# surftemp/cae_tools

Hardware: AMD Instinct MI355X
Metric: train images/sec (16x16->256x256, batch 64) (higher is better)
Workload: dtype f32

## Files before the change

cae_tools_amd/_lib.py:

```python
import ctypes as C
import os

_HERE = os.path.dirname(os.path.abspath(__file__))
LIB_PATH = os.path.join(_HERE, "csrc", "libcae_hip.so")


class CaeError(RuntimeError):
    pass


class LayerSpecC(C.Structure):
    _fields_ = [(n, C.c_int32) for n in ("in_c", "in_h", "in_w", "out_c", "out_h", "out_w", "k_h", "k_w",
                                          "stride", "output_padding")]


class TensorInfoC(C.Structure):
    _fields_ = [("name", C.c_char * 96), ("arena", C.c_int32), ("ndim", C.c_int32), ("shape", C.c_int64 * 4),
                ("offset", C.c_int64), ("numel", C.c_int64)]


class ProfileRecC(C.Structure):
    _fields_ = [("name", C.c_char * 48), ("layer", C.c_int32), ("reserved", C.c_int32), ("micros", C.c_double),
                ("bytes", C.c_double)]

# ... 35 lines not shown
    "cae_adam_step": (C.c_int, [_P]),
    "cae_forward_backward_sync": (C.c_int, [_P, C.c_int, _P, C.c_int, C.c_int, C.c_int, ALLREDUCE_FN, _P]),
    "cae_dp_unique_id": (C.c_int, [_P]),
    "cae_dp_init": (C.c_int, [_P, C.c_int, C.c_int, _P]),
    "cae_dp_shutdown": (C.c_int, [_P]),
    "cae_dp_info": (C.c_int, [_P, C.POINTER(C.c_int), C.POINTER(C.c_int), C.POINTER(C.c_int)]),
    "cae_dp_set_overlap": (C.c_int, [_P, C.c_int]),
    "cae_dp_broadcast_state": (C.c_int, [_P, C.c_int, C.c_int]),
    "cae_dp_train_step": (C.c_int, [_P, C.c_int, _P, C.c_int, C.c_int, C.c_int]),
    "cae_dp_train_steps": (C.c_int, [_P, C.c_int, _P, C.c_int, C.c_int, C.c_int, C.c_int]),
    "cae_dp_eval_steps": (C.c_int, [_P, C.c_int, _P, C.c_int, C.c_int, C.c_int]),
    "cae_dp_read_losses": (C.c_int, [_P, C.c_int, C.c_int, C.POINTER(C.c_double)]),
    "cae_eval_step": (C.c_int, [_P, C.c_int, _P, C.c_int]),
    "cae_score": (C.c_int, [_P, _P, C.c_int, _P]),
    "cae_encode": (C.c_int, [_P, _P, C.c_int, _P]),
    "cae_decode": (C.c_int, [_P, _P, C.c_int, _P]),
    "cae_read_losses": (C.c_int, [_P, C.c_int, C.c_int, C.POINTER(C.c_double)]),
    "cae_loss_slots": (C.c_int, [_P]),
    "cae_sync": (C.c_int, [_P]),
    "cae_graph_count": (C.c_int, [_P]),
    "cae_graph_captures": (C.c_int64, [_P]),
    "cae_debug_read": (C.c_int64, [_P, C.c_char_p, C.c_int, _P, C.c_int64]),
    "cae_debug_plan": (C.c_int, [_P, C.c_int, C.c_int, C.c_char_p, C.c_int64]),
    "cae_profile_begin": (C.c_int, [_P]),
    "cae_debug_launch_floor": (C.c_int, [_P, C.c_int, C.POINTER(C.c_double)]),
    "cae_profile_end": (C.c_int, [_P, C.POINTER(ProfileRecC), C.c_int]),
    "cae_trace_range_push": (C.c_int, [C.c_char_p]),
    "cae_trace_range_pop": (C.c_int, []),
    "cae_scan_f32": (C.c_int, [_P, C.c_int64, _P, C.POINTER(C.c_double)]),
    "cae_normalise_pack": (C.c_int, [_P, C.c_int64, C.c_int, C.c_int64, _P, C.c_int, C.c_int, C.c_float,
                                     C.c_float, C.c_int, _P]),
    "cae_normalise_pack_rows": (C.c_int, [_P, C.c_int64, C.c_int, C.c_int64, _P, C.c_int, C.c_int, C.c_float,
                                          C.c_float, C.c_int, _P, _P]),
    "cae_invert_permutation": (C.c_int, [_P, C.c_int64, _P, _P]),
    "cae_denormalise_f64": (C.c_int, [_P, C.c_int64, C.c_double, C.c_double, _P, _P]),
    "cae_bswap32": (C.c_int, [_P, C.c_int64, _P]),
    "cae_metric_sums": (C.c_int, [_P, _P, _P, C.c_int64, C.c_int64, C.c_double, C.c_double, _P, _P]),
    "cae_case_measures_workspace_bytes": (C.c_int64, [C.c_int64, C.c_int64]),
    "cae_case_measures": (C.c_int, [_P, C.c_int, C.c_int64, _P, C.c_int, C.c_int64, C.c_int64, C.c_int64, _P, _P,
                                    C.c_int64, _P]),
    "cae_case_range_workspace_bytes": (C.c_int64, [C.c_int64, C.c_int64]),
    "cae_case_range": (C.c_int, [_P, C.c_int, C.c_int64, _P, C.c_int, C.c_int64, C.c_int64, C.c_int64, _P, _P, C.c_int64,
                                 _P]),
    "cae_render_cases": (C.c_int, [_P, C.c_int, C.c_int64, _P, C.c_int, C.c_int64, _P, C.c_int64, C.c_int64, C.c_int64,
                                   C.c_int64, C.c_double, C.c_double, C.c_int, _P, _P]),
    "cae_pixel_sums_workspace_bytes": (C.c_int64, [C.c_int64, C.c_int64, C.c_int64]),
# ... 142 lines not shown
```

cae_tools_amd/csrc/engine.hip:

```cpp
#include <hip/hip_runtime.h>

#include <dlfcn.h>

#include <algorithm>
#include <cmath>
#include <cstdio>
#include <cstdlib>
#include <cstring>
#include <map>
#include <string>
#include <tuple>
#include <vector>

#include "cae_hip.h"
#include "kernels_generic.h"
#include "kernels_stateless.h"
#include "kernels_spectra.h"
#include "kernels_ssim.h"
#include "kernels_baseline.h"
#include "kernels_hist.h"
#include "kernels_strata.h"
#include "kernels_fss.h"
#include "kernels_s2.h"
#include "kernels_last.h"
// ... 209 lines not shown
    for (auto& L : e->dec)
        if (L.has_bn) e->bn_saved_off[L.bn_index] = carve((int64_t)L.cout * 2 * sizeof(float));
    const int64_t mb = max_batch;
    for (auto& L : e->enc) {
        L.act_off = carve(mb * L.out_elems() * 4);
        L.grad_off = carve(mb * L.out_elems() * 4);
    }
    for (int i = 0; i < 4; i++) {
        e->fc[i].act_off = carve(mb * e->fc[i].nout * 4);
        e->fc[i].grad_off = carve(mb * e->fc[i].nout * 4);
    }
    for (auto& L : e->dec) {
        if (!L.has_bn) continue;
        L.act_off = carve(mb * L.out_elems() * 4);
        L.grad_off = carve(mb * L.out_elems() * 4);
    }
    e->off_glast = carve(mb * e->dec.back().out_elems() * 4);
    e->off_xbatch = carve((mb * e->enc[0].in_elems() + e->enc[0].cout) * 4);
    if (variational) {
        e->off_vz = carve(mb * latent_size * 4);
        e->off_vgz = carve(mb * latent_size * 4);
        e->off_zlast = carve(mb * e->dec.back().out_elems() * 4);
    }
    e->ws_need = carve.top;
    for (auto& L : e->enc)
        if (L.cin > e->max_channels) e->max_channels = L.cin;
    for (auto& L : e->dec)
        if (L.cin > e->max_channels) e->max_channels = L.cin;
    if (lds_bytes(e->max_channels, e->max_channels) > 60 * 1024) {
        delete e;
        return fail(CAE_ERR_ARG, "channel count %d exceeds the LDS constant table", e->max_channels);
    }
    *out = e;
    return CAE_OK;
}

void cae_engine_destroy(cae_engine* e) {
    if (!e) return;
    e->drop_graphs();
    (void)cae_dp_shutdown(e);
    delete e;
}

int64_t cae_param_count(const cae_engine* e) { return e ? e->tab.n_param : 0; }
int64_t cae_buffer_count(const cae_engine* e) { return e ? e->tab.n_buf : 0; }
int cae_tensor_count(const cae_engine* e) { return e ? e->tab.count() : 0; }
// ... 28 lines not shown
        e->lr_stale = true;
    }
    e->stream = (hipStream_t)hip_stream;
    return CAE_OK;
}

int cae_set_graph_mode(cae_engine* e, int enabled) {
    if (!e) return fail(CAE_ERR_ARG, "null engine");
    e->graph_mode = enabled != 0;
    if (!e->graph_mode) e->drop_graphs();
    return CAE_OK;
}

int cae_set_capture_only(cae_engine* e, int enabled) {
    if (!e) return fail(CAE_ERR_ARG, "null engine");
    e->capture_only = enabled != 0;
    return CAE_OK;
}

int cae_set_kernel_mode(cae_engine* e, int specialised) {
    if (!e) return fail(CAE_ERR_ARG, "null engine");
    const int ctb = (specialised & 2) ? 0x7fffffff : e->ctbwd_auto;
    const bool gather = (specialised & 4) != 0;
    if (e->use_s2 != ((specialised & 1) != 0) || ctb != e->ctbwd_mask || gather != e->gather_fwd) e->drop_graphs();
    e->use_s2 = (specialised & 1) != 0;
    e->ctbwd_mask = ctb;
    e->gather_fwd = gather;
    return CAE_OK;
}

int cae_set_hyper(cae_engine* e, double lr, double beta1, double beta2, double eps, double weight_decay) {
    if (!e) return fail(CAE_ERR_ARG, "null engine");
    Hyper h{lr, beta1, beta2, eps, weight_decay};
    if (h.beta1 != e->hp.beta1 || h.beta2 != e->hp.beta2 || h.eps != e->hp.eps || h.wd != e->hp.wd) e->drop_graphs();
    e->hp = h;
    e->lr_stale = true;
    return push_lr(e);
}

int cae_set_lr(cae_engine* e, double lr) {
    if (!e) return fail(CAE_ERR_ARG, "null engine");
    e->hp.lr = lr;
    e->lr_stale = true;
    return push_lr(e);
}

int cae_set_dataset(cae_engine* e, int which, const float* x, const float* t, int64_t n) {
    if (!e || which < 0 || which > 1 || !x || n < 1) return fail(CAE_ERR_ARG, "cae_set_dataset: bad argument");
    if (e->ds_x[which] != x || e->ds_t[which] != t) e->drop_graphs();
    e->ds_x[which] = x;
// ... 619 lines not shown
```

cae_tools_amd/csrc/engine_choose.h:

```cpp
#pragma once

namespace {


#define S2_SHAPES(X) X(2, 1) X(4, 2) X(8, 4) X(6, 3)
#define S2_KERNELS(X, CI, CO) X(CI, CO, 3, 3) X(CI, CO, 4, 4) X(CI, CO, 3, 4) X(CI, CO, 4, 3)

template <int CI, int CO, int KH, int KW>
struct S2Shape { static constexpr int cin = CI, cout = CO, kh = KH, kw = KW; };

template <class F>
auto s2_for_shape(const ConvLayer& L, F fn) {
#define ONE(CI, CO, KH_, KW_) \
    if (L.cin == CI && L.cout == CO && L.kh == KH_ && L.kw == KW_) return fn(S2Shape<CI, CO, KH_, KW_>{});
#define PAIR(CI, CO) S2_KERNELS(ONE, CI, CO)
    S2_SHAPES(PAIR)
#undef PAIR
#undef ONE
    return false;
}

bool s2_shape_ok(const ConvLayer& L) { return L.transposed && L.stride == 2 && s2_for_shape(L, [](auto) { return true; }); }

bool s2_eligible(const cae_engine* e, const ConvLayer& L) { return e->use_s2 && L.sh_w >= 0 && s2_shape_ok(L); }
// ... 413 lines not shown
    if (rows_ok(e, L, l)) return DF_ROWS;
    if (s2_eligible(e, L)) return DF_S2;
    if (e->use_s2 && !last && L.stride == 2 && L.kh <= 4 && L.kw <= 4) {
        CtFwd c;
        int waves = 0;
        size_t lds = 0;
        return ct_fwd_plan(e, B, L, l, c, waves, lds) ? DF_CT_LDS : DF_IG;
    }
    return DF_UP;
}

DecBwdK choose_dec_bwd(const cae_engine* e, const ConvLayer& L, int l, int B, bool external_loss) {
    const bool last = l + 1 == (int)e->dec.size();
    if (last && !external_loss && last_fused_ok(e, L)) return DB_FUSED_LAST;
    if (rows_ok(e, L, l)) return DB_ROWS;
    if (s2_eligible(e, L)) return DB_S2;
    if (e->use_s2) {
        CtBwdPlan p;
        return ct_bwd_plan(e, B, L, l, p) ? DB_CT_LDS : DB_IG;
    }
    return DB_GENERIC;
}

bool enc_conv0_fits_adam(const cae_engine* e, const StepArgs& a, const ConvLayer& L) {
    return e->use_s2 && !a.syncing() && a.world == 1 && L.cout <= 64 &&
           (int64_t)L.cin * L.cout * L.kh * L.kw <= 4096 && (int64_t)a.batch * L.hout * L.wout < kDivSmallMaxN &&
           L.hout * L.wout < kDivSmallMaxD && L.in_elems() < (1 << 24) && L.out_elems() < (1 << 24) &&
           (int64_t)a.batch * L.in_elems() < (1 << 30) && (int64_t)a.batch * L.out_elems() < (1 << 30) &&
           e->bn_stat_off[L.bn_index] == e->off_zero_begin;
}

bool enc_conv0_in_adam_ok(const cae_engine* e, const StepArgs& a, const ConvLayer& L) {
    return a.adam_follows && e->x_published && enc_conv0_fits_adam(e, a, L);
}

bool linear_bwd_burst(const cae_engine* e, int i) {
    const int K = e->fc[i].nout;
    return i > 0 && K % 4 == 0 && K >= 128 && (K / 4 + 3) / 4 <= kBurstSteps;
}

const char* head_staging(const HeadArgs& h) {
    const int per = h.enc[0].cin * h.enc[0].hin * h.enc[0].win;
    if (per & 3) return "scalar";
    return h.B * (per >> 2) <= 4 * kHeadThreads ? "direct" : "gather4";
}

// ... 105 lines not shown
                     t.sp_d[2].per, t.sp_w[0].lg, t.sp_w[0].per, t.sp_w[1].lg, t.sp_w[1].per, t.sp_w[2].lg, t.sp_w[2].per, lds);
        } else {
            snprintf(line, sizeof line, "tail bwd=layers why=%s\n", why);
        }
        s += line;
        for (int i = 3; tr && !tail_fused && i >= 0; i--) {
            if (e->use_s2) snprintf(line, sizeof line, "fc%d bwd=pair burst=%d\n", i, (int)linear_bwd_burst(e, i));
            else snprintf(line, sizeof line, "fc%d bwd=generic\n", i);
            s += line;
        }
    }
    if (tr) {
        const bool in_adam = head_fused && enc_conv0_fits_adam(e, a, e->enc[0]);
        snprintf(line, sizeof line, "enc conv0=%s inner=%s\n", in_adam ? "adam" : "own",
                 e->enc.size() < 2 ? "-" : (e->use_s2 && !a.syncing() ? "pair" : "layers"));
        s += line;
    }
    if ((int64_t)s.size() + 1 > out_bytes)
        return fail(CAE_ERR_ARG, "cae_debug_plan: the report needs %zu bytes, got %lld", s.size() + 1, (long long)out_bytes);
    memcpy(out, s.c_str(), s.size() + 1);
    return CAE_OK;
}

}
```

cae_tools_amd/csrc/engine_launch.h:

```cpp
#pragma once

namespace {


template <class K, class A>
void s2_go(K kernel, A a, int ex, int ey, int tw, int th, int cap, hipStream_t s) {
    a.tiles_x = (ex + tw - 1) / tw;
    a.tiles_y = (ey + th - 1) / th;
    a.total_tiles = a.B * a.tiles_x * a.tiles_y;
    hipLaunchKernelGGL(kernel, dim3(a.total_tiles < cap ? a.total_tiles : cap), dim3(256), 0, s, a);
}

template <int CIN, int COUT, int KH, int KW>
bool s2_fwd_launch(const S2Fwd& a, S2FwdPick p, hipStream_t s) {
    const int px = ((a.OW + 1) / 2 + 1) / 2, py = ((a.OH + 1) / 2 + 1) / 2;
    const int qx = (a.OW + 1) / 2, qy = (a.OH + 1) / 2;
    switch (p.k) {
        case S2F_CS:
            if constexpr (CIN * COUT * KH * KW > 80 && (256 / COUT) % 64 == 0) {
                constexpr int PIX = 256 / COUT;
                if (p.tw == 64) s2_go(k_s2_fwd_cs<CIN, COUT, KH, KW, 64>, a, qx, qy, 64, PIX / 64, kS2FwdCap, s);
                else s2_go(k_s2_fwd_cs<CIN, COUT, KH, KW, 32>, a, qx, qy, 32, PIX / 32, kS2FwdCap, s);
                return true;
            }
// ... 287 lines not shown
    const ConvLayer& L = c.L;
    S2Last f = zeroed<S2Last>();
    f.B = a.batch; f.H = L.hin; f.W = L.win; f.OH = L.hout; f.OW = L.wout;
    f.in = c.ain.p; f.w = e->params + L.w_off; f.bias = e->params + L.b_off;
    f.target = e->ds_t[a.which]; f.perm = a.perm; f.use_cursor = a.use_cursor ? 1 : 0;
    f.st = e->state(); f.losses = e->losses();
    f.inv_count = (float)(1.0 / ((double)a.global_batch * L.cout * L.hout * L.wout));
    f.bias_acc = e->sgacc() + L.sh_b; f.wacc = e->sgacc() + L.sh_w; f.acc_stride = e->segs.n;
    f.bn_in = c.prod.P ? bn_of(e, *c.prod.P, BN_BATCH, (double)a.bn_batch * c.prod.P->hout * c.prod.P->wout, 1) : bn_none();
    f.gin = c.prod.gin; f.stats_in = c.prod.stats_in;
    ProfScope _p(e, "s2_convt_last_fused", c.l, bytes_bwd(a.batch, L, true, false));
    return last_fused_dispatch(L, f, e->stream) ? CAE_OK : fail(CAE_ERR_STATE, "decoder layer %d: no k_s2_last_fused kernel for the chosen variant", c.l);
}

void bwd_rows(cae_engine* e, const StepArgs& a, const ConvBwd& c) {
    const ConvLayer& L = c.L;
    S2Rows f = zeroed<S2Rows>();
    f.B = a.batch; f.H = L.hin; f.W = L.win; f.OH = L.hout; f.OW = L.wout;
    f.g = c.gy.p; f.yout = c.gy.q; f.bn_out = c.bng;
    f.ain = c.ain.p; f.bn_in = c.prod.bn_prev;
    f.w = e->params + L.w_off; f.wacc = e->sgacc() + L.sh_w; f.wacc_stride = e->segs.n;
    f.gin = c.prod.gin; f.stats_in = c.prod.stats_in;
    f.bg = bn_grad_out(e, L, a);
    ProfScope _p(e, "s2_convt_bwd", c.l, bytes_bwd(a.batch, L, false, false));
    rows_bwd_launch(L, f, e->stream);
}

int bwd_s2(cae_engine* e, const StepArgs& a, const ConvBwd& c) {
    const ConvLayer& L = c.L;
    S2Bwd f = zeroed<S2Bwd>();
    f.B = a.batch; f.H = L.hin; f.W = L.win; f.OH = L.hout; f.OW = L.wout;
    f.g = c.gy.p; f.yout = c.gy.q; f.bn_out = c.bng;
    f.ain = c.ain.p; f.bn_in = c.prod.bn_prev;
    f.w = e->params + L.w_off; f.wacc = e->sgacc() + L.sh_w; f.wacc_stride = e->segs.n;
    f.gin = c.prod.gin; f.stats_in = c.prod.stats_in;
    f.bg = bn_grad_out(e, L, a);
    ProfScope _p(e, "s2_convt_bwd", c.l, bytes_bwd(a.batch, L, c.last, false));
    return s2_bwd_dispatch(L, f, e->stream) ? CAE_OK : fail(CAE_ERR_STATE, "decoder layer %d: no k_s2_bwd kernel for the chosen variant", c.l);
}

int bwd_ct_lds(cae_engine* e, const StepArgs& a, const ConvBwd& c) {
    const ConvLayer& L = c.L;
    CtBwdPlan cp;
    (void)ct_bwd_plan(e, a.batch, L, c.l, cp);
    CtBwd f = zeroed<CtBwd>();
    f.B = a.batch; f.Cin = L.cin; f.H = L.hin; f.W = L.win; f.Cout = L.cout; f.OH = L.hout; f.OW = L.wout;
    f.imgs = cp.imgs; f.wstr = cp.wstr; f.bands = cp.bands; f.hb = cp.hb;
    f.g = c.gy.p; f.yout = c.gy.q; f.bn_out = c.bng;
    f.ain = c.ain.p; f.bn_in = c.prod.bn_prev;
    f.w = e->params + L.w_off;
    f.wacc = L.sh_w >= 0 ? e->sgacc() + L.sh_w : e->gradacc() + L.w_off;
    f.wacc_stride = L.sh_w >= 0 ? e->segs.n : 0;
    f.gin = c.prod.gin; f.stats_prev = c.prod.stats_in;
    f.bg = bn_grad_out(e, L, a);
    ProfScope _p(e, "ct_convt_bwd", c.l, bytes_bwd(a.batch, L, c.last, c.l == 0));
    if (cae_internal::ctbwd_launch(&f, sizeof f, (unsigned)cp.groups, (unsigned)(L.cin / 16), (unsigned)cp.parts, cp.lds_launch, e->stream))
        return fail(CAE_ERR_ARG, "k_ct_bwd_lds: argument layout mismatch");
    return CAE_OK;
}

void bwd_ig(cae_engine* e, const StepArgs& a, const ConvBwd& c) {
    const ConvLayer& L = c.L;
    const int B = a.batch;
    const IgBwdPlan p = ig_bwd_plan(L, B);
    IgWgrad fw = zeroed<IgWgrad>();
    fw.B = B; fw.Cin = L.cin; fw.H = L.hin; fw.W = L.win; fw.Cout = L.cout; fw.OH = L.hout; fw.OW = L.wout;
    fw.KH = L.kh; fw.KW = L.kw; fw.S = L.stride;
    fw.ain = c.ain.p; fw.bn_in = c.prod.bn_prev; fw.g = c.gy.p; fw.yout = c.gy.q; fw.bn_out = c.bng;
    fw.wacc = e->gradacc() + L.w_off;
    fw.bg = bn_grad_out(e, L, a);
    fw.ksteps_per_block = p.per;
    IgDgrad fd = zeroed<IgDgrad>();
    fd.B = B; fd.Cin = L.cin; fd.H = L.hin; fd.W = L.win; fd.Cout = L.cout; fd.OH = L.hout; fd.OW = L.wout;
    fd.KH = L.kh; fd.KW = L.kw; fd.S = L.stride;
    fd.g = c.gy.p; fd.yout = c.gy.q; fd.bn_out = c.bng; fd.w = e->params + L.w_off;
    fd.gin = c.prod.gin; fd.yprev = c.prod.yprev; fd.bn_prev = c.prod.bn_prev; fd.stats_prev = c.prod.stats_in;
    fd.ksplit = p.ksplit; fd.tiles_per_wave = p.tiles_per_wave;
// ... 59 lines not shown
        gd.epi = GE_STORE;
    } else if (i > 0) {
        const FcLayer& G = e->fc[i - 1];
        gd.C = e->fptr(G.grad_off); gd.H = e->fptr(G.act_off);
        gd.epi = G.relu ? GE_RELU_MASK : GE_STORE;
    } else {
        gd.C = e->fptr(P.grad_off); gd.H = e->fptr(P.act_off);
        gd.epi = GE_BN_MASK; gd.bn_c = bni; gd.hw_c = hw; gd.stats_c = e->bn_stats(P.bn_index);
        lds = gemm_lds(P.cout);
    }
    const int tiles_d = ((gd.M + 15) / 16) * ((gd.N + 15) / 16);
    if (i == 0) {
        gw.M = F.nin + 1; gw.N = F.nout; gw.K = B;
        gw.A = in; gw.sa_m = 1; gw.sa_k = F.nin;
        gw.B = gout; gw.sb_k = F.nout; gw.sb_n = 1;
        gw.epi = GE_ACC64_T; gw.ones_col = 0; gw.ones_row = 1;
        gw.bn_a = bni; gw.hw_a = hw; gw.bn_a_by_row = 1;
    }
    {
        const int tiles_w = ((gw.M + 15) / 16) * ((gw.N + 15) / 16);
        ProfScope _p(e, "linear_bwd_pair_mfma", i, bytes_lin_bwd_pair(B, F));
        const bool burst = linear_bwd_burst(e, i);
        if (burst && gemm16_burst_lds(gd.K) > lds) lds = gemm16_burst_lds(gd.K);
        hipLaunchKernelGGL(k_gemm16_pair, dim3(tiles_w + tiles_d), dim3(256), lds, e->stream, gw, gd, tiles_w, burst ? 1 : 0);
    }
    if (i == 2 && e->variational) {
        if (!e->hooks.reparam_bwd) return fail(CAE_ERR_STATE, "trunk engine without a reparameterisation hook");
        e->hooks.reparam_bwd(e->hooks.user, e->stream, e->fptr(e->off_vgz), e->fptr(e->fc[1].act_off), B, e->latent,
                             e->fptr(e->fc[1].grad_off));
    }
    return CAE_OK;
}

void linear_bwd_generic(cae_engine* e, const StepArgs& a, int i, const ConvLayer& P) {
    const FcLayer& F = e->fc[i];
    const int B = a.batch, hw = P.hout * P.wout;
    hipStream_t s = e->stream;
    const float* gout = e->fptr(F.grad_off);
    const float* in = linear_in(e, i, P);
    BnDesc bni = i == 0 ? bn_of(e, P, BN_SAVED, 0, 0) : bn_none();
    {
        ProfScope _p(e, "linear_wgrad", i, f4((double)B * (F.nin + F.nout)) + 8.0 * F.nin * F.nout);
        hipLaunchKernelGGL(k_lin_wgrad, dim3(grid1((int64_t)F.nin * F.nout)), dim3(256),
                           lds_bytes(i == 0 ? P.cout : 0, 0), s, B, F.nin, F.nout, gout, in, bni, hw,
                           e->gradacc() + F.w_off, e->gradacc() + F.b_off);
    }
    ProfScope _p(e, "linear_dgrad", i, f4((double)B * (2.0 * F.nin + F.nout) + (double)F.nin * F.nout));
// ... 66 lines not shown
```

cae_tools_amd/csrc/engine_state.h:

```cpp
#pragma once

namespace {

constexpr float kBnEps = 1e-5f;
constexpr float kBnMomentum = 0.1f;
constexpr int kLossSlots = 1 << 16;

int64_t align_up(int64_t v, int64_t a) { return (v + a - 1) / a * a; }

template <class T>
T zeroed() {
    T t;
    memset(&t, 0, sizeof t);
    return t;
}

struct ConvLayer {
    bool transposed;
    int cin, hin, win, cout, hout, wout, kh, kw, stride, opad;
    bool has_bn;
    int bn_index;
    int64_t w_off, b_off, gamma_off, beta_off;
    int64_t rm_off, rv_off;
    int64_t act_off, grad_off;
// ... 29 lines not shown
    int64_t ws_need = 0;

    float *params = nullptr, *grads = nullptr, *m = nullptr, *v = nullptr, *bufs = nullptr;
    char* ws = nullptr;
    hipStream_t stream = nullptr;
    Hyper hp{1e-3, 0.9, 0.999, 1e-8, 1e-5};
    const float* ds_x[2] = {nullptr, nullptr};
    const float* ds_t[2] = {nullptr, nullptr};
    int64_t ds_n[2] = {0, 0};
    bool graph_mode = true;
    bool lr_stale = true;
    long long captures = 0;
    bool capture_only = false;
    bool use_s2 = true;
    bool variational = false;
    int64_t off_vz = 0, off_vgz = 0, off_zlast = 0;
    cae_internal::TrunkHooks hooks{nullptr, nullptr, nullptr};
    bool gather_fwd = false;
    int ctbwd_mask = 0;
    int ctbwd_auto = 0;
    int64_t off_xbatch = 0;
    bool x_published = false;
    AdamConv0 c0_pending{};
    bool profiling = false;
    struct ProfRec { const char* name; int layer; double bytes; hipEvent_t e0, e1; };
    std::vector<ProfRec> prof;
    std::map<std::tuple<int, int, int, int, const void*, int, int, int, int, int>, hipGraphExec_t> graphs;

    int dp_world = 0, dp_rank = 0;
    RcclApi::comm_t dp_comm = nullptr;
    hipStream_t comm_stream = nullptr;
    hipEvent_t ev_fork = nullptr, ev_join = nullptr;
    bool dp_graph_ok = true;
    bool dp_overlap = true;
    std::vector<int> sync_order;
    size_t sync_pos = 0;
    int64_t bucket_split = 0;

    StepState* state() const { return reinterpret_cast<StepState*>(ws + off_state); }
    double* losses() const { return reinterpret_cast<double*>(ws + off_losses); }
    double* gradacc() const { return reinterpret_cast<double*>(ws + off_gradacc); }
    double* sgacc() const { return reinterpret_cast<double*>(ws + off_sgacc); }
    ShardSegs shard_segs() const {
        ShardSegs r = segs;
        r.base = sgacc();
        return r;
// ... 221 lines not shown
```

cae_tools_amd/csrc/kernels_ctbwd.h:

```cpp
#pragma once
#include <type_traits>

#include "device_common.h"

namespace cae {

struct CtBwd {
    int B, Cin, H, W, Cout, OH, OW;
    int imgs;
    int bands, hb;
    int wstr;
    const float* g;
    const float* yout;
    BnDesc bn_out;
    const float* ain;
    BnDesc bn_in;
    const float* w;
    float* gin;
    double* stats_prev;
    double* wacc;
    long long wacc_stride;
    BnGradOut bg;
};

constexpr int kCtbThreads = 512;
constexpr int kCtbWaves = kCtbThreads / 64;
constexpr int kCtbG4 = 7;
constexpr int kCtbA4 = 2;
constexpr int kCtbW4 = 3;
constexpr int kCtbKChunk = 64;

inline size_t ct_bwd_lds_bytes(int Cin, int Cout, int imgs, int HW, int OHW, int wstr) {
    size_t floats = 32 * (size_t)kCtbWaves;
    floats += 4 * (size_t)(Cin + Cout);
    floats += (size_t)imgs * Cout * OHW;
    floats += (size_t)imgs * 16 * HW;
    floats += 16 * (size_t)wstr;
    floats += 3 * (size_t)imgs * HW;
    floats += (size_t)kCtbWaves * 16 * 17;
    return (floats + 8) * sizeof(float);
}

#ifdef CAE_CTBWD_KERNEL
template <bool BAND>
__device__ __forceinline__ void ct_bwd_body(const CtBwd& a) {
// ... 240 lines not shown
                    ok[u] = p < pend;
                    const int pc = ok[u] ? p : pbeg;
                    ia[u] = pos_a[pc];
                    ig[u] = pos_g[pc];
                }
                float va[8], vb[8];
#pragma unroll
                for (int u = 0; u < 8; u++) {
                    va[u] = ar[ia[u]];
                    vb[u] = gb[ig[u]];
                }
#pragma unroll
                for (int u = 0; u < 8; u++) {
                    float x = va[u];
                    if (act) x = fmaxf(0.f, fmaf(x - kin.x, kin.y, kin.z));
                    va[u] = ok[u] ? x : 0.f;
                }
#pragma unroll
                for (int u = 0; u < 8; u += 2) {
                    acc = __builtin_amdgcn_mfma_f32_16x16x4f32(va[u], vb[u], acc, 0, 0, 0);
                    acc1 = __builtin_amdgcn_mfma_f32_16x16x4f32(va[u + 1], vb[u + 1], acc1, 0, 0, 0);
                }
            }
            if (n_ok) {
#pragma unroll
                for (int j = 0; j < 4; j++) acc_add<ACC_GRAD>(&wacc_sh[(size_t)(cb * 16 + 4 * q + j) * N + n], (double)(acc[j] + acc1[j]));
            }
        }
    }
    if (a.stats_prev) {
#pragma unroll
        for (int cc = 0; cc < 4; cc++) {
            float t1 = s1[cc], t2 = s2[cc];
            t1 += dpp_f<0xB1>(t1);  t2 += dpp_f<0xB1>(t2);
            t1 += dpp_f<0x4E>(t1);  t2 += dpp_f<0x4E>(t2);
            t1 += dpp_f<0x141>(t1); t2 += dpp_f<0x141>(t2);
            t1 += dpp_f<0x140>(t1); t2 += dpp_f<0x140>(t2);
            if (pl == 0) {
                lstat[wv * 32 + 2 * (4 * cg + cc)] = t1;
                lstat[wv * 32 + 2 * (4 * cg + cc) + 1] = t2;
            }
        }
        __syncthreads();
        if (tid < 32) {
            const int c = cb * 16 + (tid >> 1);
            const int shard = (blockIdx.x + blockIdx.y + blockIdx.z) & (kStatShards - 1);
            double t = 0.0;
// ... 19 lines not shown
```

cae_tools_amd/csrc/kernels_gemm.h:

```cpp
#pragma once
#include "device_common.h"

namespace cae {

enum GemmEpi : int {
    GE_STORE = 0,
    GE_RELU_MASK = 1,
    GE_BN_MASK = 2,
    GE_ACC64 = 3,
    GE_ACC64_T = 4
};

struct GemmArgs {
    int M, N, K;
    const float* A; long long sa_m, sa_k;
    const float* B; long long sb_k, sb_n;
    float* C; long long sc_m, sc_n;
    int epi;
    const float* bias;
    int relu;
    const float* H;
    BnDesc bn_a;
    int hw_a;
    int bn_a_by_row;
// ... 174 lines not shown
    __syncthreads();
    if (wv != 0 || cn >= g.N) return;
#pragma unroll
    for (int j = 0; j < 4; j++) {
        const int cm = tm * 16 + q * 4 + j;
        if (cm >= g.M) continue;
        float v = part[j * 64 + lane] + part[256 + j * 64 + lane] + part[512 + j * 64 + lane] + part[768 + j * 64 + lane];
        const long long off = (long long)cm * g.sc_m + (long long)cn * g.sc_n;
        if (g.epi == GE_STORE) {
            v += bias;
            if (g.relu) v = fmaxf(v, 0.f);
        } else {
            v = hmask[j] > 0.f ? v : 0.f;
        }
        g.C[off] = v;
    }
}

__global__ void __launch_bounds__(256) k_gemm16(GemmArgs g) {
    extern __shared__ double lds_d[];
    gemm16_body(g, blockIdx.x, lds_d);
}

__global__ void __launch_bounds__(256) k_gemm16_pair(GemmArgs a, GemmArgs b, int na, int b_burst) {
    kernarg_warm<2 * sizeof(GemmArgs) + 8>();
    extern __shared__ double lds_d[];
    if ((int)blockIdx.x < na) gemm16_body(a, blockIdx.x, lds_d);
    else if (b_burst) gemm16_burst_body(b, blockIdx.x - na, lds_d);
    else gemm16_body(b, blockIdx.x - na, lds_d);
}

}
```

cae_tools_amd/csrc/kernels_rows.h:

```cpp
#pragma once
#include "kernels_last.h"

namespace cae {

struct S2Rows {
    int B, H, W, OH, OW;
    int QH;
    int bands;
    int groups;
    const float* g;
    const float* yout;
    BnDesc bn_out;
    const float* ain;
    BnDesc bn_in;
    const float* w;
    float* gin;
    double* stats_in;
    double* wacc;
    int wacc_stride;
    BnGradOut bg;
};

template <int CIN, int CT, int COUT, int KH, int KW, int HB, int IMGS, int D>
__global__ void __launch_bounds__(256) __attribute__((amdgpu_waves_per_eu(1, 2))) k_s2_bwd_rows(S2Rows a) {
    kernarg_warm<sizeof(S2Rows)>();
    constexpr int CS = CIN / CT;
    constexpr int NB = 4 / CS;
    constexpr int LW = 64 / IMGS;
    constexpr int NACC = CT * COUT * KH * KW;
    constexpr int NRED = NACC + 2 * CT;
    constexpr int NR = HB + 1;
    static_assert(CS * NB == 4 && CS * CT == CIN, "four waves");
    static_assert(KH == 3 && KW == 3, "3x3 stride-2 kernels");
    static_assert(CIN <= 8 && COUT <= 8, "one lane per (channel, shard) in the BatchNorm prologue");
    __shared__ float redf[4 * NRED];
    __shared__ __attribute__((aligned(16))) float wscr[4 * kWsumScratch];
    __shared__ float xch[NB > 1 ? 4 * CT * 64 : 1];
    __shared__ __attribute__((aligned(16))) float wl[CIN * COUT * 12];

    const int tid = threadIdx.x, lane = tid & 63;
    const int wv = __builtin_amdgcn_readfirstlane(tid >> 6);
    const int cgrp = wv % CS, bsel = wv / CS;
    const int c0 = cgrp * CT;
// ... 240 lines not shown
            }
        }
    }

    {
        float red[NRED];
#pragma unroll
        for (int i = 0; i < NACC; i++) red[i] = dw[i];
#pragma unroll
        for (int c = 0; c < CT; c++) {
            red[NACC + 2 * c] = d1[c];
            red[NACC + 2 * c + 1] = d2[c];
        }
        wave_sums_lds<NRED>(red, wscr + wv * kWsumScratch, redf + wv * NRED, lane);
    }
    __syncthreads();
    const int shard = blockIdx.x & (kStatShards - 1);
    for (int i = tid; i < CS * NRED; i += 256) {
        const int gsel = i / NRED, j = i - gsel * NRED;
        double s = 0.0;
#pragma unroll
        for (int q = 0; q < NB; q++) s += (double)redf[(q * CS + gsel) * NRED + j];
        if (j < NACC) {
            acc_add<ACC_GRAD>(&a.wacc[(size_t)shard * a.wacc_stride + (size_t)gsel * NACC + j], s);
        } else {
            const int jj = j - NACC;
            acc_add<ACC_GRAD>(&a.stats_in[((size_t)shard * CIN + gsel * CT + (jj >> 1)) * 4 + 2 + (jj & 1)], s);
        }
    }
}

}

namespace cae {

struct S2FwdRows {
    int B, H, W, OH, OW;
    int QH;
    int bands, groups;
    const float* in;
    BnDesc bn_in;
    const float* w;
    const float* bias;
    float* out;
    double* stats;
};

// ... 193 lines not shown
```

cae_tools_amd/csrc/unet_engine.hip:

```cpp
#include <hip/hip_runtime.h>

#include <cmath>
#include <cstdio>
#include <cstring>
#include <algorithm>
#include <map>
#include <string>
#include <vector>

#include "cae_unet.h"
#include "engine_host.h"
#include "kernels_unet.h"
#include "kernels_unet_mfma.h"
#include "kernels_unet_lin.h"
#include "kernels_unet_thin.h"
#include "kernels_unet_patch.h"

namespace ugemm {
#include "device_common.h"
#include "kernels_gemm.h"
}

using namespace unet;
using namespace cae_internal;
// ... 362 lines not shown
            }
            hipLaunchKernelGGL(k_lin_outer, dim3((L.nin + 127) / 128, (L.nout + 127) / 128), dim3(256), lds, e->stream, gout, (long long)L.nout, in,
                               (long long)L.nin, B, L.nout, L.nin, reinterpret_cast<float*>(e->gacc(L.w)), e->gacc(L.b));
            if (gin) lin_gemm(e, false, gout, L.nout, e->P(L.w), L.nin, nullptr, gin, B, L.nin, L.nout);
            return;
        }
        case LIN_GEMM16: {
            ugemm::cae::GemmArgs gw = gemm16_args(L.nout, L.nin + 1, B);
            gw.A = gout, gw.sa_m = 1, gw.sa_k = L.nout;
            gw.B = in, gw.sb_k = L.nin, gw.sb_n = 1;
            gw.epi = ugemm::cae::GE_ACC64;
            gw.accW = e->gacc(L.w), gw.accB = e->gacc(L.b), gw.ones_col = 1;
            const int tiles_w = ((gw.M + 15) / 16) * ((gw.N + 15) / 16);
            if (!gin) {
                hipLaunchKernelGGL(ugemm::cae::k_gemm16, dim3(tiles_w), dim3(256), gemm16_lds(), e->stream, gw);
                return;
            }
            ugemm::cae::GemmArgs gd = gemm16_args(B, L.nin, L.nout);
            gd.A = gout, gd.sa_m = L.nout, gd.sa_k = 1;
            gd.B = e->P(L.w), gd.sb_k = L.nin, gd.sb_n = 1;
            gd.C = gin, gd.sc_m = L.nin, gd.sc_n = 1;
            gd.epi = ugemm::cae::GE_STORE;
            const int tiles_d = ((gd.M + 15) / 16) * ((gd.N + 15) / 16);
            hipLaunchKernelGGL(ugemm::cae::k_gemm16_pair, dim3(tiles_w + tiles_d), dim3(256), gemm16_lds(), e->stream, gw, gd, tiles_w, 0);
            return;
        }
        case LIN_TILE: {
            GemmDesc w{L.nout, L.nin, B, gout, 1, L.nout, in, L.nin, 1, nullptr, nullptr, e->gacc(L.w), L.nin, 1, 2};
            gemm_launch(w, nullptr, 0, e->stream);
            hipLaunchKernelGGL(k_col_sums, dim3((L.nout + 255) / 256), dim3(256), 0, e->stream, B, L.nout, gout, e->gacc(L.b));
            if (gin) {
                GemmDesc d{L.nin, B, L.nout, e->P(L.w), 1, L.nin, gout, 1, L.nout, nullptr, gin, nullptr, 1, L.nin, 0};
                gemm_launch(d, reinterpret_cast<float*>(e->ws + e->off_gpart), e->gpart_bytes, e->stream);
            }
            return;
        }
        case LIN_GENERIC: break;
    }
    hipLaunchKernelGGL(k_lin_wgrad, dim3(blocks_for((long long)L.nout * L.nin, 65536)), dim3(256), 0, e->stream, B, L.nin,
                       L.nout, gout, in, e->gacc(L.w), e->gacc(L.b));
    if (gin)
        hipLaunchKernelGGL(k_lin_dgrad, dim3(blocks_for((long long)B * L.nin, 65536)), dim3(256), 0, e->stream, B, L.nin,
                           L.nout, gout, e->P(L.w), gin);
}

std::vector<const ConvLayer*> pack_list(const unet_engine* e, bool train) {
    std::vector<const ConvLayer*> v;
// ... 753 lines not shown
```

cae_tools_amd/engine.py:

```python
import ctypes as C
from collections import OrderedDict

import numpy as np
import torch

from . import _lib
from ._engine_base import TEST, TRAIN, SpecPlan, _spec_layers, _to_c, require_gpu
from ._lib import CaeError, check


class EnginePlan(SpecPlan):

    PREFIX = "cae_"

    def bn_prefixes(self):
        return [n[: -len(".running_mean")] for n in self.tensors if n.endswith(".running_mean")]

    def set_kernel_mode(self, mode):
        check(self.lib.cae_set_kernel_mode(self.handle, int(mode)))

    def kernel_plan(self, batch, train):
        return self._plan_report(batch, train)


class HipEngine(EnginePlan):

    def __init__(self, spec, fc_size, latent_size, max_batch, device=None, graph=True, specialised=True):
        require_gpu()
        super().__init__(spec, fc_size, latent_size, max_batch)
        self._bind(device, grads=True, buffers=True)
        check(self.lib.cae_set_graph_mode(self.handle, 1 if graph else 0))
        check(self.lib.cae_set_kernel_mode(self.handle, int(specialised) if isinstance(specialised, int) and not isinstance(specialised, bool) else (1 if specialised else 0)))
        torch.cuda.synchronize(self.device)
        self.num_batches_tracked = 0
        self.adam_steps = 0
        self._datasets = {}
        self._keep = []
        self.loss_slots = int(self.lib.cae_loss_slots(self.handle))
        self._slot = 0
        self._cursor = None

    def grad_view(self, name):
# ... 345 lines not shown
```

include/cae_hip.h:

```cpp
#ifndef CAE_HIP_H
#define CAE_HIP_H

#include <stdint.h>

#ifdef __cplusplus
extern "C" {
#endif

typedef struct cae_engine cae_engine;

enum cae_status {
    CAE_OK = 0,
    CAE_ERR_ARG = -1,
    CAE_ERR_STATE = -2,
    CAE_ERR_HIP = -3
};

typedef struct {
    int32_t in_c, in_h, in_w;
    int32_t out_c, out_h, out_w;
    int32_t k_h, k_w;
    int32_t stride;
    int32_t output_padding;
} cae_layer_spec;
// ... 60 lines not shown
int cae_dp_broadcast_state(cae_engine* e, int root, int what);
int cae_dp_train_step(cae_engine* e, int which, const int32_t* perm_dev, int batch, int global_batch, int sync_bn);
int cae_dp_train_steps(cae_engine* e, int which, const int32_t* perm_dev, int batch, int global_batch, int sync_bn, int nsteps);
int cae_dp_eval_steps(cae_engine* e, int which, const int32_t* perm_dev, int batch, int global_batch, int nsteps);
int cae_dp_read_losses(cae_engine* e, int first, int count, double* host_out);

int cae_eval_step(cae_engine* e, int which, const int32_t* perm_dev, int batch);

int cae_score(cae_engine* e, const float* x_dev, int batch, float* y_dev);

int cae_encode(cae_engine* e, const float* x_dev, int batch, float* z_dev);
int cae_decode(cae_engine* e, const float* z_dev, int batch, float* y_dev);

int cae_read_losses(cae_engine* e, int first, int count, double* host_out);
int cae_loss_slots(const cae_engine* e);
int cae_sync(cae_engine* e);
int cae_graph_count(const cae_engine* e);
int64_t cae_graph_captures(const cae_engine* e);

int64_t cae_debug_read(cae_engine* e, const char* what, int index, void* host_out, int64_t capacity_elems);

int cae_debug_plan(const cae_engine* e, int batch, int train, char* out_host, int64_t out_bytes);


typedef struct {
    char name[48];
    int32_t layer;
    int32_t reserved;
    double micros;
    double bytes;
} cae_profile_rec;
int cae_profile_begin(cae_engine* e);
int cae_debug_launch_floor(cae_engine* e, int n, double* micros_per_kernel);
int cae_profile_end(cae_engine* e, cae_profile_rec* out, int capacity);

int cae_trace_range_push(const char* name);
int cae_trace_range_pop(void);


int cae_scan_f32(const float* x_dev, int64_t n, void* hip_stream, double* out3_host);

int cae_normalise_pack(const float* src_dev, int64_t n, int c_src, int64_t hw, float* dst_dev,
                       int c_dst, int c_off, float vmin, float range, int enable, void* hip_stream);

int cae_normalise_pack_rows(const float* src_dev, int64_t n, int c_src, int64_t hw, float* dst_dev, int c_dst, int c_off,
                            float vmin, float range, int enable, const int32_t* dst_row_dev, void* hip_stream);
// ... 146 lines not shown
```

Baseline: 391,600.

## Replace decoder weight-grad atomics with per-block slabs folded in the linear backward kernel

In the s2 decoder backward kernels (rows and ct_lds), each block now writes its partial weight-gradient values to a dedicated workspace slab instead of doing atomic adds into the f64 accumulator. The partials are then reduced by extra workgroups prepended to the last linear layer's k_gemm16_pair launch, which runs later in the backward pass, so the fold overlaps the GEMM. This removes atomic contention on small weight tensors and makes the sum order deterministic. In exchange it adds workspace memory, host-side slab-table computation on every launch, and extra global traffic for writing and re-reading the partials. A kernel-mode bit can switch back to atomics.

```diff
diff --git a/cae_tools_amd/_lib.py b/cae_tools_amd/_lib.py
--- a/cae_tools_amd/_lib.py
+++ b/cae_tools_amd/_lib.py
@@ -81,6 +81,7 @@
     "cae_graph_captures": (C.c_int64, [_P]),
     "cae_debug_read": (C.c_int64, [_P, C.c_char_p, C.c_int, _P, C.c_int64]),
     "cae_debug_plan": (C.c_int, [_P, C.c_int, C.c_int, C.c_char_p, C.c_int64]),
+    "cae_debug_wgrad_slabs": (C.c_int, [_P, C.c_int, C.c_char_p, C.c_int64]),
     "cae_profile_begin": (C.c_int, [_P]),
     "cae_debug_launch_floor": (C.c_int, [_P, C.c_int, C.POINTER(C.c_double)]),
     "cae_profile_end": (C.c_int, [_P, C.POINTER(ProfileRecC), C.c_int]),
diff --git a/cae_tools_amd/csrc/engine.hip b/cae_tools_amd/csrc/engine.hip
--- a/cae_tools_amd/csrc/engine.hip
+++ b/cae_tools_amd/csrc/engine.hip
@@ -255,6 +255,8 @@
         e->off_vgz = carve(mb * latent_size * 4);
         e->off_zlast = carve(mb * e->dec.back().out_elems() * 4);
     }
+    e->wslab_bytes = wgrad_slab_capacity(e);
+    e->off_wslab = carve(std::max<int64_t>(e->wslab_bytes, 256));
     e->ws_need = carve.top;
     for (auto& L : e->enc)
         if (L.cin > e->max_channels) e->max_channels = L.cin;
@@ -329,10 +331,13 @@
     if (!e) return fail(CAE_ERR_ARG, "null engine");
     const int ctb = (specialised & 2) ? 0x7fffffff : e->ctbwd_auto;
     const bool gather = (specialised & 4) != 0;
-    if (e->use_s2 != ((specialised & 1) != 0) || ctb != e->ctbwd_mask || gather != e->gather_fwd) e->drop_graphs();
+    const bool atomics = (specialised & 8) != 0;
+    if (e->use_s2 != ((specialised & 1) != 0) || ctb != e->ctbwd_mask || gather != e->gather_fwd || atomics != e->wgrad_atomics)
+        e->drop_graphs();
     e->use_s2 = (specialised & 1) != 0;
     e->ctbwd_mask = ctb;
     e->gather_fwd = gather;
+    e->wgrad_atomics = atomics;
     return CAE_OK;
 }
 
diff --git a/cae_tools_amd/csrc/engine_choose.h b/cae_tools_amd/csrc/engine_choose.h
--- a/cae_tools_amd/csrc/engine_choose.h
+++ b/cae_tools_amd/csrc/engine_choose.h
@@ -459,6 +459,89 @@
     return DB_GENERIC;
 }
 
+bool wgrad_slabs_on(const cae_engine* e) { return e->use_s2 && !e->wgrad_atomics; }
+
+struct WSlab { int layer; const char* writer; int nvals, nparts, f64, kfull, ppg; int64_t off; };
+
+void ct_bwd_slab(const ConvLayer& L, const CtBwdPlan& p, int B, WSlab& s) {
+    auto chunks = [](int positions) { return (positions + kCtbKChunk - 1) / kCtbKChunk; };
+    s.nvals = L.cin * L.cout * 9;
+    s.f64 = 0;
+    if (p.bands > 1) {
+        s.writer = "ct_bwd_band";
+        s.kfull = chunks(p.hb * L.win);
+        s.ppg = (p.bands - 1) * s.kfull + chunks((L.hin - (p.bands - 1) * p.hb) * L.win);
+        s.nparts = p.groups * s.ppg;
+    } else {
+        s.writer = "ct_bwd_lds";
+        s.kfull = s.ppg = chunks(p.imgs * L.hin * L.win);
+        s.nparts = (p.groups - 1) * s.kfull + chunks((B - (p.groups - 1) * p.imgs) * L.hin * L.win);
+    }
+}
+
+int rows_bwd_grid(const ConvLayer& L, int B) {
+    const RowsPick p = choose_rows_bwd(L);
+    const int qh = (L.hout + 1) / 2, hmax = L.hin > qh - 1 ? L.hin : qh - 1, nb = L.cin == 4 ? 4 : 1;
+    const int bands = (hmax + p.hb - 1) / p.hb, imgs = 64 / p.lw;
+    return ((B + imgs - 1) / imgs) * ((bands + nb - 1) / nb);
+}
+
+std::vector<WSlab> wgrad_slab_table(const cae_engine* e, int B, bool external_loss, int64_t capacity) {
+    std::vector<WSlab> t;
+    if (!wgrad_slabs_on(e)) return t;
+    int64_t used = 0;
+    for (int l = (int)e->dec.size() - 1; l >= 0; l--) {
+        const ConvLayer& L = e->dec[l];
+        WSlab s{l, "", L.cin * L.cout * L.kh * L.kw, 0, 1, 0, 0, 0};
+        switch (choose_dec_bwd(e, L, l, B, external_loss)) {
+            case DB_ROWS:
+                s.writer = "s2_bwd_rows"; s.nparts = rows_bwd_grid(L, B);
+                break;
+            case DB_CT_LDS: {
+                CtBwdPlan p;
+                (void)ct_bwd_plan(e, B, L, l, p);
+                ct_bwd_slab(L, p, B, s);
+                break;
+            }
+            default: continue;
+        }
+        const int64_t bytes = align_up((int64_t)s.nparts * s.nvals * (s.f64 ? 8 : 4), 256);
+        if ((int)t.size() >= kFoldMax || used + bytes > capacity) continue;
+        s.off = used;
+        used += bytes;
+        t.push_back(s);
+    }
+    return t;
+}
+
+WSlab wgrad_slab_of(const cae_engine* e, int B, bool external_loss, int l) {
+    for (const WSlab& s : wgrad_slab_table(e, B, external_loss, e->wslab_bytes))
+        if (s.layer == l) return s;
+    return WSlab{l, "", 0, 0, 0, 0, 0, 0};
+}
+
+int64_t wgrad_slab_capacity(cae_engine* e) {
+    const int mask = e->ctbwd_mask;
+    e->ctbwd_mask = 0x7fffffff;
+    int64_t cap = 0;
+    for (int B = 1; B <= e->max_batch; B++) {
+        const std::vector<WSlab> t = wgrad_slab_table(e, B, e->variational, INT64_MAX / 2);
+        if (!t.empty()) cap = std::max(cap, t.back().off + align_up((int64_t)t.back().nparts * t.back().nvals * (t.back().f64 ? 8 : 4), 256));
+    }
+    e->ctbwd_mask = mask;
+    return cap;
+}
+
+WFold wgrad_fold_of(const cae_engine* e, const std::vector<WSlab>& t) {
+    WFold f = zeroed<WFold>();
+    for (const WSlab& s : t) {
+        const int vshift = fold_vshift(s.nparts);
+        f.s[f.nslab++] = WFoldSlab{e->ws + e->off_wslab + s.off, e->gradacc() + e->dec[s.layer].w_off, s.nvals, s.nparts, s.f64, vshift};
+        f.nwg += fold_wgs(s.nvals, vshift);
+    }
+    return f;
+}
+
 bool enc_conv0_fits_adam(const cae_engine* e, const StepArgs& a, const ConvLayer& L) {
     return e->use_s2 && !a.syncing() && a.world == 1 && L.cout <= 64 &&
            (int64_t)L.cin * L.cout * L.kh * L.kw <= 4096 && (int64_t)a.batch * L.hout * L.wout < kDivSmallMaxN &&
@@ -610,4 +693,29 @@
     return CAE_OK;
 }
 
-}
+int cae_debug_wgrad_slabs(const cae_engine* e, int batch, char* out, int64_t out_bytes) {
+    if (!e || !out || out_bytes < 1) return fail(CAE_ERR_ARG, "cae_debug_wgrad_slabs: bad argument");
+    if (batch < 1 || batch > e->max_batch)
+        return fail(CAE_ERR_ARG, "cae_debug_wgrad_slabs: batch %d outside 1 .. %d", batch, e->max_batch);
+    const std::vector<WSlab> t = wgrad_slab_table(e, batch, e->variational, e->wslab_bytes);
+    const WFold f = wgrad_fold_of(e, t);
+    std::string s;
+    char line[256];
+    int64_t used = 0;
+    for (size_t k = 0; k < t.size(); k++) {
+        const WSlab& sl = t[k];
+        snprintf(line, sizeof line, "dec%d writer=%s type=%s param=%lld values=%d partials=%d offset=%lld fold_wgs=%d fold_values=%d\n", sl.layer,
+                 sl.writer, sl.f64 ? "f64" : "f32", (long long)e->dec[sl.layer].w_off, sl.nvals, sl.nparts, (long long)sl.off,
+                 fold_wgs(sl.nvals, f.s[k].vshift), 1 << f.s[k].vshift);
+        s += line;
+        used = sl.off + (int64_t)sl.nparts * sl.nvals * (sl.f64 ? 8 : 4);
+    }
+    snprintf(line, sizeof line, "fold slabs=%d wgs=%d bytes=%lld capacity=%lld\n", f.nslab, f.nwg, (long long)used, (long long)e->wslab_bytes);
+    s += line;
+    if ((int64_t)s.size() + 1 > out_bytes)
+        return fail(CAE_ERR_ARG, "cae_debug_wgrad_slabs: the report needs %zu bytes, got %lld", s.size() + 1, (long long)out_bytes);
+    memcpy(out, s.c_str(), s.size() + 1);
+    return CAE_OK;
+}
+
+}
diff --git a/cae_tools_amd/csrc/engine_launch.h b/cae_tools_amd/csrc/engine_launch.h
--- a/cae_tools_amd/csrc/engine_launch.h
+++ b/cae_tools_amd/csrc/engine_launch.h
@@ -333,6 +333,8 @@
     f.w = e->params + L.w_off; f.wacc = e->sgacc() + L.sh_w; f.wacc_stride = e->segs.n;
     f.gin = c.prod.gin; f.stats_in = c.prod.stats_in;
     f.bg = bn_grad_out(e, L, a);
+    const WSlab sl = wgrad_slab_of(e, a.batch, a.external_loss, c.l);
+    if (sl.nparts) f.wslab = reinterpret_cast<double*>(e->ws + e->off_wslab + sl.off);
     ProfScope _p(e, "s2_convt_bwd", c.l, bytes_bwd(a.batch, L, false, false));
     rows_bwd_launch(L, f, e->stream);
 }
@@ -364,6 +366,11 @@
     f.wacc_stride = L.sh_w >= 0 ? e->segs.n : 0;
     f.gin = c.prod.gin; f.stats_prev = c.prod.stats_in;
     f.bg = bn_grad_out(e, L, a);
+    const WSlab sl = wgrad_slab_of(e, a.batch, a.external_loss, c.l);
+    if (sl.nparts) {
+        f.wslab = reinterpret_cast<float*>(e->ws + e->off_wslab + sl.off);
+        f.slab_kfull = sl.kfull; f.slab_ppg = sl.ppg;
+    }
     ProfScope _p(e, "ct_convt_bwd", c.l, bytes_bwd(a.batch, L, c.last, c.l == 0));
     if (cae_internal::ctbwd_launch(&f, sizeof f, (unsigned)cp.groups, (unsigned)(L.cin / 16), (unsigned)cp.parts, cp.lds_launch, e->stream))
         return fail(CAE_ERR_ARG, "k_ct_bwd_lds: argument layout mismatch");
@@ -469,7 +476,8 @@
         ProfScope _p(e, "linear_bwd_pair_mfma", i, bytes_lin_bwd_pair(B, F));
         const bool burst = linear_bwd_burst(e, i);
         if (burst && gemm16_burst_lds(gd.K) > lds) lds = gemm16_burst_lds(gd.K);
-        hipLaunchKernelGGL(k_gemm16_pair, dim3(tiles_w + tiles_d), dim3(256), lds, e->stream, gw, gd, tiles_w, burst ? 1 : 0);
+        const WFold fold = i == 3 ? wgrad_fold_of(e, wgrad_slab_table(e, B, a.external_loss, e->wslab_bytes)) : zeroed<WFold>();
+        hipLaunchKernelGGL(k_gemm16_pair, dim3(fold.nwg + tiles_w + tiles_d), dim3(256), lds, e->stream, gw, gd, tiles_w, burst ? 1 : 0, fold);
     }
     if (i == 2 && e->variational) {
         if (!e->hooks.reparam_bwd) return fail(CAE_ERR_STATE, "trunk engine without a reparameterisation hook");
diff --git a/cae_tools_amd/csrc/engine_state.h b/cae_tools_amd/csrc/engine_state.h
--- a/cae_tools_amd/csrc/engine_state.h
+++ b/cae_tools_amd/csrc/engine_state.h
@@ -75,6 +75,8 @@
     int64_t off_xbatch = 0;
     bool x_published = false;
     AdamConv0 c0_pending{};
+    bool wgrad_atomics = false;
+    int64_t off_wslab = 0, wslab_bytes = 0;
     bool profiling = false;
     struct ProfRec { const char* name; int layer; double bytes; hipEvent_t e0, e1; };
     std::vector<ProfRec> prof;
diff --git a/cae_tools_amd/csrc/kernels_ctbwd.h b/cae_tools_amd/csrc/kernels_ctbwd.h
--- a/cae_tools_amd/csrc/kernels_ctbwd.h
+++ b/cae_tools_amd/csrc/kernels_ctbwd.h
@@ -21,6 +21,9 @@
     double* wacc;
     long long wacc_stride;
     BnGradOut bg;
+    float* wslab;
+    int slab_kfull;
+    int slab_ppg;
 };
 
 constexpr int kCtbThreads = 512;
@@ -307,7 +310,12 @@
                     acc1 = __builtin_amdgcn_mfma_f32_16x16x4f32(va[u + 1], vb[u + 1], acc1, 0, 0, 0);
                 }
             }
-            if (n_ok) {
+            if (n_ok && a.wslab) {
+                const int part = (int)blockIdx.x * a.slab_ppg + (BAND ? (int)blockIdx.z * a.slab_kfull : 0) + kc;
+                float* sl = a.wslab + (size_t)part * a.Cin * N;
+#pragma unroll
+                for (int j = 0; j < 4; j++) sl[(size_t)(cb * 16 + 4 * q + j) * N + n] = acc[j] + acc1[j];
+            } else if (n_ok) {
 #pragma unroll
                 for (int j = 0; j < 4; j++) acc_add<ACC_GRAD>(&wacc_sh[(size_t)(cb * 16 + 4 * q + j) * N + n], (double)(acc[j] + acc1[j]));
             }
diff --git a/cae_tools_amd/csrc/kernels_gemm.h b/cae_tools_amd/csrc/kernels_gemm.h
--- a/cae_tools_amd/csrc/kernels_gemm.h
+++ b/cae_tools_amd/csrc/kernels_gemm.h
@@ -220,12 +220,82 @@
     gemm16_body(g, blockIdx.x, lds_d);
 }
 
-__global__ void __launch_bounds__(256) k_gemm16_pair(GemmArgs a, GemmArgs b, int na, int b_burst) {
-    kernarg_warm<2 * sizeof(GemmArgs) + 8>();
+constexpr int kFoldMax = 6;
+constexpr int kFoldBurst = 16;
+
+struct WFoldSlab {
+    const void* slab;
+    double* acc;
+    int nvals, nparts;
+    int f64, vshift;
+};
+struct WFold {
+    int nwg;
+    int nslab;
+    WFoldSlab s[kFoldMax];
+};
+
+inline int fold_vshift(int nparts) {
+    int vshift = 8;
+    while (vshift > 3 && (256 >> vshift) * kFoldBurst < nparts) vshift--;
+    return vshift;
+}
+__host__ __device__ inline int fold_wgs(int nvals, int vshift) { return (nvals + (1 << vshift) - 1) >> vshift; }
+
+template <class T>
+__device__ __forceinline__ double wgrad_fold_column(const T* col, int first, int step, int nparts, int nvals) {
+    double sum = 0.0;
+    for (int p0 = first; p0 < nparts; p0 += step * kFoldBurst) {
+        T x[kFoldBurst];
+#pragma unroll
+        for (int u = 0; u < kFoldBurst; u++) x[u] = col[(size_t)min(p0 + step * u, nparts - 1) * nvals];
+#pragma unroll
+        for (int u = 0; u < kFoldBurst; u++) asm volatile("" : "+v"(x[u]));
+#pragma unroll
+        for (int u = 0; u < kFoldBurst; u++)
+            if (p0 + step * u < nparts) sum += acc_grid<ACC_GRAD>((double)x[u]);
+    }
+    return sum;
+}
+
+__device__ __forceinline__ void wgrad_fold_body(const WFold& f, const int bx, double* lds_d) {
+    WFoldSlab s = f.s[0];
+    int t = bx;
+    bool found = false;
+#pragma unroll
+    for (int k = 0; k < kFoldMax; k++) {
+        const int tiles = k < f.nslab ? fold_wgs(f.s[k].nvals, f.s[k].vshift) : 0;
+        if (!found && t < tiles) {
+            s = f.s[k];
+            found = true;
+        } else if (!found) {
+            t -= tiles;
+        }
+    }
+    const int tid = threadIdx.x, vals = 1 << s.vshift, groups = 256 >> s.vshift;
+    const int v = tid & (vals - 1), pg = tid >> s.vshift;
+    const int val = (t << s.vshift) + v, vc = min(val, s.nvals - 1);
+    lds_d[tid] = s.f64 ? wgrad_fold_column(static_cast<const double*>(s.slab) + vc, pg, groups, s.nparts, s.nvals)
+                       : wgrad_fold_column(static_cast<const float*>(s.slab) + vc, pg, groups, s.nparts, s.nvals);
+    __syncthreads();
+    if (tid < vals && val < s.nvals) {
+        double sum = 0.0;
+        for (int g = 0; g < groups; g++) sum += lds_d[(g << s.vshift) + tid];
+        s.acc[val] = sum;
+    }
+}
+
+__global__ void __launch_bounds__(256) k_gemm16_pair(GemmArgs a, GemmArgs b, int na, int b_burst, WFold f) {
+    kernarg_warm<2 * sizeof(GemmArgs) + 8 + sizeof(WFold)>();
     extern __shared__ double lds_d[];
-    if ((int)blockIdx.x < na) gemm16_body(a, blockIdx.x, lds_d);
-    else if (b_burst) gemm16_burst_body(b, blockIdx.x - na, lds_d);
-    else gemm16_body(b, blockIdx.x - na, lds_d);
-}
-
-}
+    if ((int)blockIdx.x < f.nwg) {
+        wgrad_fold_body(f, blockIdx.x, lds_d);
+        return;
+    }
+    const int bx = (int)blockIdx.x - f.nwg;
+    if (bx < na) gemm16_body(a, bx, lds_d);
+    else if (b_burst) gemm16_burst_body(b, bx - na, lds_d);
+    else gemm16_body(b, bx - na, lds_d);
+}
+
+}
diff --git a/cae_tools_amd/csrc/kernels_rows.h b/cae_tools_amd/csrc/kernels_rows.h
--- a/cae_tools_amd/csrc/kernels_rows.h
+++ b/cae_tools_amd/csrc/kernels_rows.h
@@ -19,6 +19,7 @@
     double* wacc;
     int wacc_stride;
     BnGradOut bg;
+    double* wslab;
 };
 
 template <int CIN, int CT, int COUT, int KH, int KW, int HB, int IMGS, int D>
@@ -305,7 +306,8 @@
 #pragma unroll
         for (int q = 0; q < NB; q++) s += (double)redf[(q * CS + gsel) * NRED + j];
         if (j < NACC) {
-            acc_add<ACC_GRAD>(&a.wacc[(size_t)shard * a.wacc_stride + (size_t)gsel * NACC + j], s);
+            if (a.wslab) a.wslab[(size_t)blockIdx.x * (CS * NACC) + gsel * NACC + j] = s;
+            else acc_add<ACC_GRAD>(&a.wacc[(size_t)shard * a.wacc_stride + (size_t)gsel * NACC + j], s);
         } else {
             const int jj = j - NACC;
             acc_add<ACC_GRAD>(&a.stats_in[((size_t)shard * CIN + gsel * CT + (jj >> 1)) * 4 + 2 + (jj & 1)], s);
diff --git a/cae_tools_amd/csrc/unet_engine.hip b/cae_tools_amd/csrc/unet_engine.hip
--- a/cae_tools_amd/csrc/unet_engine.hip
+++ b/cae_tools_amd/csrc/unet_engine.hip
@@ -408,7 +408,8 @@
             gd.C = gin, gd.sc_m = L.nin, gd.sc_n = 1;
             gd.epi = ugemm::cae::GE_STORE;
             const int tiles_d = ((gd.M + 15) / 16) * ((gd.N + 15) / 16);
-            hipLaunchKernelGGL(ugemm::cae::k_gemm16_pair, dim3(tiles_w + tiles_d), dim3(256), gemm16_lds(), e->stream, gw, gd, tiles_w, 0);
+            hipLaunchKernelGGL(ugemm::cae::k_gemm16_pair, dim3(tiles_w + tiles_d), dim3(256), gemm16_lds(), e->stream, gw, gd, tiles_w, 0,
+                               ugemm::cae::WFold{});
             return;
         }
         case LIN_TILE: {
diff --git a/cae_tools_amd/engine.py b/cae_tools_amd/engine.py
--- a/cae_tools_amd/engine.py
+++ b/cae_tools_amd/engine.py
@@ -18,6 +18,15 @@
 
     def set_kernel_mode(self, mode):
         check(self.lib.cae_set_kernel_mode(self.handle, int(mode)))
+
+    def wgrad_slabs(self, batch):
+        buf = C.create_string_buffer(1 << 14)
+        check(self.lib.cae_debug_wgrad_slabs(self.handle, int(batch), buf, len(buf)))
+        report = {}
+        for line in buf.value.decode().splitlines():
+            (name, *fields) = line.split()
+            report[name] = dict(f.split("=", 1) for f in fields)
+        return report
 
     def kernel_plan(self, batch, train):
         return self._plan_report(batch, train)
diff --git a/include/cae_hip.h b/include/cae_hip.h
--- a/include/cae_hip.h
+++ b/include/cae_hip.h
@@ -106,6 +106,8 @@
 
 int cae_debug_plan(const cae_engine* e, int batch, int train, char* out_host, int64_t out_bytes);
 
+int cae_debug_wgrad_slabs(const cae_engine* e, int batch, char* out_host, int64_t out_bytes);
+
 
 typedef struct {
     char name[48];
```

Measured after the change: 397,400 (median of 6 runs). +1.5%, better.
